# Farmadupe/vid_dup_finder_lib

Measured on AMD Instinct MI355X. Metric: hash-pairs/sec all-pairs Hamming (search(), tolerance 0.35) [+ frames/sec DCT-hash in 'summary.hash_summary'], higher is better.
Workload: dtype fp4 e2m1 ({0,1}) x fp4 -> f32 accumulate (exact half-integers < 2^11)

## Files before the change

### vid_dup_finder_lib_amd/csrc/api.cpp

```cpp
#include <algorithm>
#include <chrono>
#include <cmath>
#include <cstdio>
#include <cstdlib>
#include <cstring>
#include <memory>
#include <numeric>

#include "host_sort.h"
#include "vdf_ctx.h"

namespace {
thread_local std::string g_create_error;
inline double now_ms() { return std::chrono::duration<double, std::milli>(std::chrono::steady_clock::now().time_since_epoch()).count(); }
}

vdf_ctx::~vdf_ctx()
{
    if (!subs.empty() || !workers.empty()) vdf_impl::destroy_multi(this);
    if (copy_pool) vdf_impl::destroy_copy_pool(this);
    for (auto &kv : axis_tables) {
        kv.second->start.release(); kv.second->size.release(); kv.second->w.release();
        delete kv.second;
    }
    for (auto &kv : mfma_tables) {
        kv.second->operand.release(); kv.second->bias.release(); kv.second->meta.release();
        delete kv.second;
    }
    for (auto &kv : box_tables) {
        kv.second->blob.release(); kv.second->entries.release();
        delete kv.second;
    }
    DevBuf *all[] = {&row_lo, &row_hi, &tile_lo, &tile_hi, &tile_first, &tile_count, &tile_offset, &counters,
                     &hits, &perm, &matched, &exp_cols, &exp_rows, &pop_cols, &pop_rows, &cand, &group_cmin, &group_offset, &group_blocks, &up_hashes,
                     &up_dur, &up_ref_hashes, &up_ref_dur, &small, &frames, &frames2, &out_hashes, &out_hashes2, &out_dc,
                     &out_dc2, &cos_table, &crops, &crop_desc, &crop_tables, &crop_desc2, &crop_tables2, &crop_work, &sort_scratch, &sort_scratch_pub, &hits2, &hit_bitmaps, &bitmap_gather};
    for (DevBuf *b : all) b->release();
    for (PinBuf &b : pin) b.release();
    for (PinBuf &b : pin_out) b.release();
    pin_small.release();
    pin_ctrl.release();
    pin_crops.release();
    pin_desc.release();
    host_hits.buf.release();
    if (ev0) (void)hipEventDestroy(ev0);
    if (ev1) (void)hipEventDestroy(ev1);
    if (ev_mid) (void)hipEventDestroy(ev_mid);
    if (ev_wait) (void)hipEventDestroy(ev_wait);
    for (hipEvent_t e : ev_copy) if (e) (void)hipEventDestroy(e);
    for (hipEvent_t e : ev_done) if (e) (void)hipEventDestroy(e);
    if (copy_stream) (void)hipStreamDestroy(copy_stream);
    if (stream) (void)hipStreamDestroy(stream);
}

namespace vdf_impl {

void set_create_error(const std::string &msg) { g_create_error = msg; }

int fail(vdf_ctx *ctx, int code, const std::string &msg)
{
    if (ctx) ctx->err = msg;
    return code;
}

int fail_hip(vdf_ctx *ctx, hipError_t e, const char *what)
{
    std::string msg = std::string(what) + ": " + hipGetErrorString(e);
    (void)hipGetLastError();
    return fail(ctx, e == hipErrorOutOfMemory ? VDF_E_OOM : VDF_E_HIP, msg);
}

bool is_sorted_u32(const uint32_t *d, size_t n)
{
    for (size_t i = 1; i < n; i++)
        if (d[i] < d[i - 1]) return false;
    return true;
}

constexpr size_t kPinSmallBytes = 4u << 20;
constexpr uint64_t kDeviceSortHits = 1u << 17;
constexpr uint32_t kRefsMinWorkgroups = 2048;
constexpr uint64_t kSpecSortHits = 1u << 14;
constexpr uint64_t kFilterHits = 1u << 16;

int search_core(vdf_ctx *ctx, int mode, const uint64_t *d_col_hashes, const uint32_t *d_col_dur, size_t n_cols,
                const uint64_t *d_row_hashes, const uint32_t *d_row_dur, const uint32_t *d_row_perm, size_t n_rows,
                uint32_t tol_int, uint32_t shard_index, uint32_t shard_count, uint32_t row_begin, uint32_t row_end,
                const uint32_t *d_matched, uint32_t row_index_base, vdf_hit *hits, uint64_t capacity,
                uint64_t *n_hits_out, uint32_t *overflow_row_out, hipStream_t stream, bool replay_only, vdf_ctx::HostHits *staging,
                ShardExchange *fx)
{
    *n_hits_out = 0;
    *overflow_row_out = 0xFFFFFFFFu;
    if (n_rows == 0 || n_cols == 0) return VDF_OK;
    if (n_rows >= 0xFFFFFFFFull || n_cols >= 0xFFFFFFFFull) return fail(ctx, VDF_E_INVAL, "more than 2^32-1 hashes");
    if (shard_count == 0 || shard_index >= shard_count) return fail(ctx, VDF_E_INVAL, "bad shard index/count");
    VDF_HIP(ctx, hipSetDevice(ctx->device));
    const double t_enter = now_ms();

    vdf::SearchLaunch L{};
    const bool mfma = ctx->search_backend == 1;
    L.tile_rows = mfma ? (mode == 1 ? ctx->mfma_refs_rows : ctx->mfma_self_rows) : ctx->tile_rows;
    L.chunk_cols = mfma ? ctx->mfma_chunk_cols : ctx->chunk_cols;
    L.n_row_tiles = (uint32_t)((n_rows + L.tile_rows - 1) / L.tile_rows);
    if (mfma && L.chunk_cols == 0) {
        L.chunk_cols = 65536;
        while (L.chunk_cols > 4096 && (uint64_t)L.n_row_tiles * ((n_cols + L.chunk_cols - 1) / L.chunk_cols) < ctx->mfma_min_wgs) L.chunk_cols /= 2;
    }
    while ((uint64_t)L.n_row_tiles * ((n_cols + L.chunk_cols - 1) / L.chunk_cols) >= 0x40000000ull && L.chunk_cols < (1u << 22))
        L.chunk_cols *= 2;
    const size_t padded_rows = (size_t)L.n_row_tiles * L.tile_rows;
    VDF_HIP(ctx, ctx->row_lo.reserve(padded_rows * 4));
    VDF_HIP(ctx, ctx->row_hi.reserve(padded_rows * 4));
    VDF_HIP(ctx, ctx->tile_lo.reserve((size_t)L.n_row_tiles * 4));
    VDF_HIP(ctx, ctx->tile_hi.reserve((size_t)L.n_row_tiles * 4));
    VDF_HIP(ctx, ctx->tile_first.reserve((size_t)L.n_row_tiles * 4));
    VDF_HIP(ctx, ctx->tile_count.reserve((size_t)L.n_row_tiles * 4));
    VDF_HIP(ctx, ctx->tile_offset.reserve(((size_t)L.n_row_tiles + 1) * 4));
    VDF_HIP(ctx, ctx->counters.reserve(64));
    const uint64_t dev_cap = std::max<uint64_t>(capacity, 1);
    VDF_HIP(ctx, ctx->hits.reserve(dev_cap * sizeof(vdf_hit)));

    L.row_hashes = reinterpret_cast<const uint32_t *>(d_row_hashes);
    L.row_perm = d_row_perm;
    L.n_rows = (uint32_t)n_rows;
    L.row_index_base = row_index_base;
    L.col_hashes = reinterpret_cast<const uint32_t *>(d_col_hashes);
    L.n_cols = (uint32_t)n_cols;
    L.row_lo = ctx->row_lo.as<uint32_t>();
    L.row_hi = ctx->row_hi.as<uint32_t>();
    L.tile_lo = ctx->tile_lo.as<uint32_t>();
    L.tile_hi = ctx->tile_hi.as<uint32_t>();
    L.tile_first = ctx->tile_first.as<uint32_t>();
    L.tile_count = ctx->tile_count.as<uint32_t>();
    L.tile_offset = ctx->tile_offset.as<uint32_t>();
    L.tol = tol_int;
    L.matched = d_matched;
    L.self_mode = (mode == 0);
    L.shard_index = shard_index;
    L.shard_count = shard_count;
    L.hits = ctx->hits.as<vdf_hit>();
    L.capacity = capacity;
    L.counters = ctx->counters.as<unsigned long long>();
    L.overflow_row = reinterpret_cast<uint32_t *>(ctx->counters.as<unsigned long long>() + 4);

    L.prune_step = 16;
    if (ctx->mfma_prune_step >= 0) {
        L.prune_step = ctx->mfma_prune_step;
    } else {
        for (int st = 6; st <= 14; st++) {
            const double bits = 64.0 * (st + 1);
            if (bits / 2 - 2.0 * std::sqrt(bits) >= (double)tol_int + 1) { L.prune_step = st; break; }
        }
    }
    if (mfma) L.prune_step = L.prune_step <= 6 ? 6 : L.prune_step <= 8 ? 8 : L.prune_step <= 10 ? 10 : L.prune_step <= 14 ? L.prune_step : 16;
    else L.prune_step = L.prune_step <= 6 ? 6 : L.prune_step <= 10 ? 10 : L.prune_step <= 12 ? 12 : 16;
    if (mfma) {
        L.group_size = std::min<uint32_t>(ctx->mfma_group, L.n_row_tiles);
        L.n_groups = (L.n_row_tiles + L.group_size - 1) / L.group_size;
        if (L.n_groups > 1024) return fail(ctx, VDF_E_INVAL, "too many row-tile groups");
        VDF_HIP(ctx, ctx->group_cmin.reserve((size_t)L.n_groups * 4));
        VDF_HIP(ctx, ctx->group_offset.reserve(((size_t)L.n_groups + 1) * 4));
        VDF_HIP(ctx, ctx->group_blocks.reserve((size_t)L.n_groups * 4));
        L.group_blocks = ctx->group_blocks.as<uint32_t>();
        L.group_cmin = ctx->group_cmin.as<uint32_t>();
        L.group_offset = ctx->group_offset.as<uint32_t>();
        const uint32_t k_steps = (uint32_t)(L.prune_step < 15 ? L.prune_step + 1 : 16);
        const uint32_t col_pad = (uint32_t)((n_cols + vdf::kMfmaRowPad - 1) / vdf::kMfmaRowPad * vdf::kMfmaRowPad) + vdf::kMfmaColPad;
        VDF_HIP(ctx, ctx->exp_cols.reserve((size_t)col_pad * 512));
        VDF_HIP(ctx, ctx->pop_cols.reserve((size_t)col_pad * 12));
        const ExpOwner want_owner{d_col_hashes, n_cols, k_steps, ctx->exp_cols.p};
        const bool reuse = ctx->pinned_db == d_col_hashes && ctx->pinned_n == n_cols && ctx->exp_owner == want_owner;
        if (!reuse) {
            ctx->exp_owner = ExpOwner{};
            VDF_HIP(ctx, vdf::launch_expand_fp4(L.col_hashes, (uint32_t)n_cols, col_pad, ctx->exp_cols.p, k_steps,
                                                ctx->pop_cols.as<float>(), stream));
            ctx->exp_owner = want_owner;
        }
        L.col_exp = ctx->exp_cols.p;
        L.col_pop3 = ctx->pop_cols.as<float>();
        L.col_pad = col_pad;
        if (d_row_hashes == d_col_hashes) {
            L.row_exp = ctx->exp_cols.p;
            L.row_pop3 = L.col_pop3;
            L.row_pad = col_pad;
        } else {
            const uint32_t row_pad = (uint32_t)((padded_rows + 127) / 128 * 128);
            VDF_HIP(ctx, ctx->exp_rows.reserve((size_t)row_pad * 512));
            VDF_HIP(ctx, ctx->pop_rows.reserve((size_t)row_pad * 12));
            VDF_HIP(ctx, vdf::launch_expand_fp4(L.row_hashes, (uint32_t)n_rows, row_pad, ctx->exp_rows.p, k_steps,
                                                ctx->pop_rows.as<float>(), stream));
            L.row_exp = ctx->exp_rows.p;
            L.row_pop3 = ctx->pop_rows.as<float>();
            L.row_pad = row_pad;
        }
    }
    const unsigned long long init[8] = {0, 0, 0, 0, 0xFFFFFFFFull, 0, 0, 0};
    const bool pin_ok = ctx->pin_small.reserve(kPinSmallBytes) && ctx->pin_small.pinned;
    uint64_t spec = std::min<uint64_t>(capacity, std::max<uint64_t>(ctx->hits_guess + ctx->hits_guess / 4 + 1024, 8192));
    if (!pin_ok || spec * sizeof(vdf_hit) > kPinSmallBytes) spec = 0;
    const bool spec_sort = spec && ctx->hits_guess >= kSpecSortHits;
    if (spec_sort) VDF_HIP(ctx, hipMemsetAsync(ctx->hits.p, 0xFF, (size_t)spec * sizeof(vdf_hit), stream));
    const bool adapt_refs = mode == 1 && mfma && ctx->mfma_chunk_cols == 0;
    if (adapt_refs && ctx->refs_hint_cols == n_cols && ctx->refs_hint_rows == n_rows && ctx->refs_hint_chunk) L.chunk_cols = ctx->refs_hint_chunk;
    if (!ctx->pin_ctrl.reserve(256)) return fail(ctx, VDF_E_OOM, "pinned staging");
    unsigned long long *pre = ctx->pin_ctrl.as<unsigned long long>() + 8;
    uint32_t total_tiles = 0;
    unsigned long long unsorted = 0, admitted = 0;
    for (int pass = 0;; pass++) {
        VDF_HIP(ctx, hipMemcpyAsync(ctx->counters.p, init, sizeof init, hipMemcpyHostToDevice, stream));
        VDF_HIP(ctx, vdf::launch_windows_tiles(mode, d_col_dur, (uint32_t)n_cols, d_row_dur, d_row_perm, (uint32_t)n_rows,
                                               row_begin, row_end, shard_index, shard_count, L, stream));
        VDF_HIP(ctx, hipMemcpyAsync(pre, L.counters, 64, hipMemcpyDeviceToHost, stream));
        VDF_HIP(ctx, hipMemcpyAsync(pre + 8, mfma ? L.group_offset + L.n_groups : L.tile_offset + L.n_row_tiles, 4,
                                    hipMemcpyDeviceToHost, stream));
        VDF_HIP(ctx, hipMemcpyAsync(pre + 9, L.tile_offset + L.n_row_tiles, 4, hipMemcpyDeviceToHost, stream));
        VDF_HIP(ctx, hipStreamSynchronize(stream));
        total_tiles = *reinterpret_cast<const uint32_t *>(pre + 8);
        const uint32_t busy_tiles = *reinterpret_cast<const uint32_t *>(pre + 9);
        unsorted = pre[5];
        admitted = pre[2];
        if (!adapt_refs || pass > 0 || unsorted || busy_tiles == 0 || busy_tiles >= kRefsMinWorkgroups || L.chunk_cols <= 4096) break;
        uint64_t est = busy_tiles;
        while (L.chunk_cols > 4096 && est < kRefsMinWorkgroups) { L.chunk_cols /= 2; est *= 2; }
    }
    if (adapt_refs) { ctx->refs_hint_cols = n_cols; ctx->refs_hint_rows = n_rows; ctx->refs_hint_chunk = L.chunk_cols; }
    if (unsorted) return fail(ctx, VDF_E_INVAL, "durations are not ascending: pass the arrays in Search::sort order");
    if (total_tiles >= 0x7FFFFFFFu) return fail(ctx, VDF_E_INVAL, "tile count exceeds the grid limit");
    if (mfma) {
        const uint64_t want = ((uint64_t)((double)admitted * 6e-6) + (uint64_t)total_tiles * 8 * 8 + std::max<uint64_t>(capacity, 1ull << 20)) * ctx->cand_scale;
        L.cand_capacity = (uint32_t)std::min<uint64_t>(want, 0x40000000ull);
        if (ctx->cand_capacity_override)
            L.cand_capacity = (uint32_t)std::min<uint64_t>((uint64_t)ctx->cand_capacity_override * ctx->cand_scale, 0x40000000ull);
        const void *before = ctx->cand.p;
        VDF_HIP(ctx, ctx->cand.reserve((size_t)L.cand_capacity * 16));
        if (ctx->cand.p != before) ctx->cand_dirty = SIZE_MAX;
        const size_t slots = ctx->cand.cap / 16;
        const size_t fill = (ctx->cand_dirty == SIZE_MAX ? slots : std::min<size_t>(slots, ctx->cand_dirty)) * 16;
        if (fill) VDF_HIP(ctx, hipMemsetAsync(ctx->cand.p, 0xFF, fill, stream));
        ctx->cand_dirty = L.cand_capacity;
        L.cand = ctx->cand.p;
        L.cand_head = ctx->counters.as<unsigned long long>() + 6;
    }

    ctx->timing.prep_ms += (float)(now_ms() - t_enter);
    VDF_HIP(ctx, hipEventRecord(ctx->ev0, stream));
    if (mfma) {
        VDF_HIP(ctx, vdf::launch_hamming_tiles_mfma2(L, total_tiles, stream));
        VDF_HIP(ctx, hipEventRecord(ctx->ev_mid, stream));
        if (total_tiles) VDF_HIP(ctx, vdf::launch_resolve_candidates(L, stream));
    } else {
        VDF_HIP(ctx, vdf::launch_hamming_tiles(L, total_tiles, stream));
        VDF_HIP(ctx, hipEventRecord(ctx->ev_mid, stream));
    }
    VDF_HIP(ctx, hipEventRecord(ctx->ev1, stream));
    if (!ctx->pin_ctrl.reserve(256)) return fail(ctx, VDF_E_OOM, "pinned staging");
    unsigned long long *fin = ctx->pin_ctrl.as<unsigned long long>();
    VDF_HIP(ctx, hipMemcpyAsync(fin, ctx->counters.p, 64, hipMemcpyDeviceToHost, stream));
    unsigned row_bits = 1;
    while (row_bits < 32 && ((uint64_t)row_index_base + n_rows) >> row_bits) row_bits++;
    unsigned col_bits = 1;
    while (col_bits < 32 && ((uint64_t)n_cols >> col_bits)) col_bits++;
    if (spec_sort) {
        VDF_HIP(ctx, ctx->sort_scratch.reserve(vdf::sort_hits_scratch_bytes((size_t)spec)));
        VDF_HIP(ctx, vdf::launch_sort_hits(ctx->hits.as<vdf_hit>(), (size_t)spec, row_bits, ctx->sort_scratch.p, ctx->sort_scratch.cap, stream, col_bits));
    }
    if (spec) VDF_HIP(ctx, hipMemcpyAsync(ctx->pin_small.p, ctx->hits.p, (size_t)spec * sizeof(vdf_hit), hipMemcpyDeviceToHost, stream));
    VDF_HIP(ctx, hipStreamSynchronize(stream));
    const double t_synced = now_ms();
    float ms = 0.f, ms_stream = 0.f;
    VDF_HIP(ctx, hipEventElapsedTime(&ms, ctx->ev0, ctx->ev1));
// ... 1465 lines not shown
```

### vid_dup_finder_lib_amd/csrc/hamming.hip

```cpp
#include <algorithm>

#include "vdf_internal.h"

namespace vdf {

constexpr uint32_t kMaxBlocksPerLaunch = 4u << 20;

typedef const __attribute__((address_space(4))) uint32_t *const_u32_ptr;

__device__ __forceinline__ uint32_t sat_u32(double x)
{
    if (!(x == x)) return 0u;
    if (x <= 0.0) return 0u;
    if (x >= 4294967295.0) return 0xFFFFFFFFu;
    return (uint32_t)x;
}

__device__ __forceinline__ uint32_t partition_point_lt(const uint32_t *__restrict__ d, uint32_t n, uint32_t v)
{
    uint32_t lo = 0, hi = n;
    while (lo < hi) {
        uint32_t mid = lo + ((hi - lo) >> 1);
        if (d[mid] < v) lo = mid + 1; else hi = mid;
    }
    return lo;
}
__device__ __forceinline__ uint32_t partition_point_le(const uint32_t *__restrict__ d, uint32_t n, uint32_t v)
{
    uint32_t lo = 0, hi = n;
    while (lo < hi) {
        uint32_t mid = lo + ((hi - lo) >> 1);
        if (d[mid] <= v) lo = mid + 1; else hi = mid;
    }
    return lo;
}

__device__ __forceinline__ uint32_t wave_min(uint32_t v)
{
#pragma unroll
    for (int o = 32; o > 0; o >>= 1) v = min(v, (uint32_t)__shfl_xor((int)v, o, 64));
    return v;
}
__device__ __forceinline__ uint32_t wave_max(uint32_t v)
{
#pragma unroll
    for (int o = 32; o > 0; o >>= 1) v = max(v, (uint32_t)__shfl_xor((int)v, o, 64));
    return v;
}

__device__ __forceinline__ void wave_append_hits(bool hit, uint32_t row, uint32_t col, vdf_hit *__restrict__ hits,
                                                 unsigned long long capacity, unsigned long long *__restrict__ counters,
                                                 uint32_t *__restrict__ overflow_row)
{
    const unsigned long long bal = __builtin_amdgcn_ballot_w64(hit);
    if (bal == 0ull) return;
    const int leader = __builtin_ctzll(bal);
    unsigned long long base = 0;
    if ((int)(threadIdx.x & 63) == leader) base = atomicAdd(&counters[0], (unsigned long long)__builtin_popcountll(bal));
    base = ((unsigned long long)(uint32_t)__shfl((int)(base >> 32), leader, 64) << 32) | (uint32_t)__shfl((int)(uint32_t)base, leader, 64);
    if (hit) {
        const unsigned long long at = base + __builtin_amdgcn_mbcnt_hi((uint32_t)(bal >> 32), __builtin_amdgcn_mbcnt_lo((uint32_t)bal, 0u));
        if (at < capacity) {
            vdf_hit hp; hp.row = row; hp.col = col;
            hits[at] = hp;
        } else {
            atomicMin(overflow_row, row);
        }
    }
}

__global__ __launch_bounds__(256) void windows_tiles_kernel(
    int mode, const uint32_t *__restrict__ col_dur, uint32_t n_cols, const uint32_t *__restrict__ row_dur,
    const uint32_t *__restrict__ row_perm, uint32_t n_rows, uint32_t row_begin, uint32_t row_end, uint32_t shard_index,
    uint32_t shard_count, uint32_t tile_rows, uint32_t chunk_cols, uint32_t *__restrict__ row_lo,
    uint32_t *__restrict__ row_hi, uint32_t *__restrict__ tile_lo, uint32_t *__restrict__ tile_hi,
    uint32_t *__restrict__ tile_first, uint32_t *__restrict__ tile_count, unsigned long long *__restrict__ counters)
{
    __shared__ uint32_t s_min[4], s_max[4];
    __shared__ unsigned long long s_pairs[4];
    const uint32_t t = blockIdx.x;
    const bool mine = (t % shard_count) == shard_index;
    uint32_t mn = 0xFFFFFFFFu, mx = 0u;
    unsigned long long pairs = 0;
    for (uint32_t q = threadIdx.x; q < tile_rows; q += 256) {
// ... 156 lines not shown
#pragma unroll
            for (int q = 0; q < 8; q++) {
                const uint4 v = rp[q];
                rw[k][4 * q + 0] = v.x; rw[k][4 * q + 1] = v.y; rw[k][4 * q + 2] = v.z; rw[k][4 * q + 3] = v.w;
            }
            if (self_mode && matched && ((matched[src >> 5] >> (src & 31)) & 1u)) { lo = 0; hi = 0; }
        } else {
#pragma unroll
            for (int q = 0; q < 32; q++) rw[k][q] = 0u;
            lo = 0; hi = 0;
        }
        rlo[k] = lo; rhi[k] = hi; rid[k] = row_index_base + src;
    }

    const_u32_ptr cols = (const_u32_ptr)(uintptr_t)col_hashes;
    uint32_t n_early = 0;
    for (uint32_t c = c_begin; c < c_end; ++c) {
        const_u32_ptr cp = cols + (size_t)c * 32;
        uint32_t d[R];
#pragma unroll
        for (int k = 0; k < R; k++) d[k] = 0u;
#pragma unroll
        for (int w = 0; w < (CHKW < 32 ? CHKW : 32); ++w) {
            const uint32_t cw = cp[w];
#pragma unroll
            for (int k = 0; k < R; k++) d[k] += __builtin_popcount(rw[k][w] ^ cw);
        }
        uint32_t m = d[0];
#pragma unroll
        for (int k = 1; k < R; k++) m = min(m, d[k]);
        if (CHKW < 32) {
            if (__builtin_amdgcn_ballot_w64(m <= tol) == 0ull) { n_early += 1; continue; }
#pragma unroll
            for (int w = CHKW; w < 32; ++w) {
                const uint32_t cw = cp[w];
#pragma unroll
                for (int k = 0; k < R; k++) d[k] += __builtin_popcount(rw[k][w] ^ cw);
            }
            m = d[0];
#pragma unroll
            for (int k = 1; k < R; k++) m = min(m, d[k]);
        }
        if (__builtin_amdgcn_ballot_w64(m <= tol) != 0ull) {
            bool col_ok = true;
            if (matched) col_ok = ((((const_u32_ptr)(uintptr_t)matched)[c >> 5] >> (c & 31)) & 1u) == 0u;
            if (col_ok) {
#pragma unroll
                for (int k = 0; k < R; k++)
                    wave_append_hits(d[k] <= tol && c >= rlo[k] && c < rhi[k], rid[k], c, hits, capacity, counters, overflow_row);
            }
        }
    }
    if (threadIdx.x == 0) atomicAdd(&counters[1], (unsigned long long)(c_end - c_begin) * TILE_ROWS);
    if (CHKW < 32 && lane == 0 && n_early) atomicAdd(&counters[3], (unsigned long long)n_early * (64u * R));
}

typedef int v8i __attribute__((ext_vector_type(8)));
typedef int v4i __attribute__((ext_vector_type(4)));
typedef float v16f __attribute__((ext_vector_type(16)));

__global__ __launch_bounds__(256) void expand_fp4_kernel(const uint32_t *__restrict__ packed, uint32_t n,
                                                        uint32_t n_pad, uint4 *__restrict__ expanded,
                                                        uint32_t k_steps, float *__restrict__ pop,
                                                        float *__restrict__ popk, float *__restrict__ popkT)
{
    for (size_t idx = (size_t)blockIdx.x * 256 + threadIdx.x; idx < (size_t)n_pad * 32;
         idx += (size_t)gridDim.x * 256) {
    const uint32_t hsh = (uint32_t)(idx >> 5), dw = (uint32_t)idx & 31u;
    uint4 out = {0u, 0u, 0u, 0u};
    uint32_t w = 0;
    if (hsh < n) {
        w = packed[idx];
        uint32_t o[4];
#pragma unroll
        for (int j = 0; j < 4; j++) {
            uint32_t x = (w >> (8 * j)) & 0xFFu;
            x = (x | (x << 12)) & 0x000F000Fu;
            x = (x | (x << 6)) & 0x03030303u;
            x = (x | (x << 3)) & 0x11111111u;
            o[j] = x << 1;
        }
        out = make_uint4(o[0], o[1], o[2], o[3]);
    }
    expanded[idx] = out;
    if (pop) {
        uint32_t pc = (uint32_t)__builtin_popcount(w), pk = (dw & 15u) < k_steps ? pc : 0u;
#pragma unroll
        for (int o = 16; o > 0; o >>= 1) { pc += (uint32_t)__shfl_xor((int)pc, o, 32); pk += (uint32_t)__shfl_xor((int)pk, o, 32); }
        if (dw == 0) {
            pop[hsh] = (float)pc;
            popk[hsh] = (float)pk;
            popkT[(size_t)(hsh >> 7) * 128 + (hsh & 31u) * 4 + ((hsh >> 5) & 3u)] = (float)pk;
        }
    }
    }
}

template <int N>
struct IntC { static constexpr int value = N; };
template <int I, int N, class F>
__device__ __forceinline__ void static_for(F &&f)
{
    if constexpr (I < N) {
        f(IntC<I>{});
        static_for<I + 1, N>(f);
    }
}

struct CandEntry {
    uint32_t row_base;
    uint32_t col;
    uint32_t mask;
    uint32_t pad;
};

__global__ __launch_bounds__(256) void resolve_candidates_kernel(
    const CandEntry *__restrict__ cand, const unsigned long long *__restrict__ cand_head, uint32_t cand_capacity,
    const uint32_t *__restrict__ row_hashes, const uint32_t *__restrict__ row_perm, uint32_t n_rows, uint32_t row_index_base,
    const uint32_t *__restrict__ col_hashes, uint32_t n_cols, const uint32_t *__restrict__ row_lo,
    const uint32_t *__restrict__ row_hi, uint32_t tol, const uint32_t *__restrict__ matched, int self_mode,
    vdf_hit *__restrict__ hits, unsigned long long capacity, unsigned long long *__restrict__ counters,
    uint32_t *__restrict__ overflow_row)
{
    const uint32_t n = (uint32_t)min(*cand_head, (unsigned long long)cand_capacity);
    const uint32_t lane = threadIdx.x & 63, wave = threadIdx.x >> 6;
    constexpr uint32_t kStage = 512;
    __shared__ vdf_hit s_stage[4][kStage];
    uint32_t staged = 0;
    auto flush = [&]() {
        if (staged == 0) return;
        __builtin_amdgcn_fence(__ATOMIC_ACQ_REL, "wavefront");
        __builtin_amdgcn_wave_barrier();
        unsigned long long base = 0;
        if (lane == 0) base = atomicAdd(&counters[0], (unsigned long long)staged);
        base = ((unsigned long long)(uint32_t)__builtin_amdgcn_readfirstlane((int)(base >> 32)) << 32) |
               (uint32_t)__builtin_amdgcn_readfirstlane((int)(uint32_t)base);
        for (uint32_t k = lane; k < staged; k += 64) {
            const vdf_hit hp = s_stage[wave][k];
            if (base + k < capacity) hits[base + k] = hp;
            else atomicMin(overflow_row, hp.row);
        }
        __builtin_amdgcn_fence(__ATOMIC_ACQ_REL, "wavefront");
        __builtin_amdgcn_wave_barrier();
        staged = 0;
    };
    for (uint32_t e0 = blockIdx.x * 256 + (threadIdx.x & ~63u); e0 < n; e0 += gridDim.x * 256) {
        const uint32_t e = e0 + lane;
        CandEntry ce;
        ce.row_base = 0xFFFFFFFFu; ce.col = 0; ce.mask = 0; ce.pad = 0;
        if (e < n) ce = cand[e];
        uint32_t m = ce.mask;
        if (ce.row_base == 0xFFFFFFFFu || ce.col >= n_cols) m = 0;
        if (m && matched && ((matched[ce.col >> 5] >> (ce.col & 31)) & 1u)) m = 0;
        uint4 cw[8];
        if (m) {
            const uint4 *cp = reinterpret_cast<const uint4 *>(col_hashes + (size_t)ce.col * 32);
#pragma unroll
            for (int q = 0; q < 8; q++) cw[q] = cp[q];
        }
        while (__builtin_amdgcn_ballot_w64(m != 0u) != 0ull) {
            bool hit = false;
            uint32_t src = 0;
            if (m) {
                const uint32_t r = (uint32_t)__builtin_ctz(m);
                m &= m - 1;
                const uint32_t p = ce.row_base + (r & 3) + 8 * (r >> 2);
                if (p < n_rows) {
                    const uint32_t lo = row_lo[p], hi = row_hi[p];
                    if (ce.col >= lo && ce.col < hi) {
                        src = row_perm ? row_perm[p] : p;
                        if (!(self_mode && matched && ((matched[src >> 5] >> (src & 31)) & 1u))) {
                            const uint4 *rp = reinterpret_cast<const uint4 *>(row_hashes + (size_t)src * 32);
                            uint32_t d = 0;
#pragma unroll
                            for (int q = 0; q < 8; q++) {
                                const uint4 v = rp[q];
                                d += __builtin_popcount(v.x ^ cw[q].x) + __builtin_popcount(v.y ^ cw[q].y) +
                                     __builtin_popcount(v.z ^ cw[q].z) + __builtin_popcount(v.w ^ cw[q].w);
                            }
                            hit = d <= tol;
                        }
                    }
                }
            }
            const unsigned long long bal = __builtin_amdgcn_ballot_w64(hit);
            if (bal == 0ull) continue;
            const uint32_t cnt = (uint32_t)__builtin_popcountll(bal);
            if (staged + cnt > kStage) flush();
            if (hit) {
                vdf_hit hp; hp.row = row_index_base + src; hp.col = ce.col;
                s_stage[wave][staged + __builtin_amdgcn_mbcnt_hi((uint32_t)(bal >> 32), __builtin_amdgcn_mbcnt_lo((uint32_t)bal, 0u))] = hp;
            }
            staged += cnt;
        }
    }
    flush();
}

template <int CHK, int WAVES>
__global__ __launch_bounds__(64 * WAVES, 2) void hamming_mfma2_kernel(
    const uint4 *__restrict__ row_exp, const uint32_t *__restrict__ row_perm, uint32_t n_rows,
    uint32_t row_index_base, const uint4 *__restrict__ col_exp, const uint32_t *__restrict__ row_lo,
    const uint32_t *__restrict__ row_hi, const uint32_t *__restrict__ tile_lo, const uint32_t *__restrict__ tile_hi,
    const uint32_t *__restrict__ tile_first, const uint32_t *__restrict__ tile_count,
    const uint32_t *__restrict__ group_offset, const uint32_t *__restrict__ group_cmin, uint32_t n_groups,
    uint32_t group_size, uint32_t shard_index, uint32_t shard_count, uint32_t n_row_tiles, uint32_t chunk_cols,
    uint32_t tol, const uint32_t *__restrict__ matched, int self_mode, vdf_hit *__restrict__ hits,
    unsigned long long capacity, unsigned long long *__restrict__ counters, uint32_t *__restrict__ overflow_row,
    uint32_t block_base, const float *__restrict__ row_pop3, uint32_t row_pad, const float *__restrict__ col_pop3,
    uint32_t col_pad, CandEntry *__restrict__ cand, uint32_t cand_capacity, unsigned long long *__restrict__ cand_head)
{
    constexpr int K = CHK < 15 ? CHK + 1 : 16;
    constexpr bool kRowcLds = K > 13;
    constexpr uint32_t kSub = WAVES >= 8 ? 4 : 2;
    constexpr uint32_t kColStep = 32 * kSub;
    constexpr int NBLK = 2 * (int)kSub;
    constexpr int NM = NBLK * K;
    constexpr int P = (K == 16 && WAVES >= 8) ? 2 : 4, NB = P + 1;
    constexpr uint32_t kTileRows = 64 * WAVES;
    constexpr int kDmaPerWave = (int)(kColStep * 32 / (64 * WAVES));
    constexpr int kDmaEvery = NM / kDmaPerWave;
    static_assert(kDmaEvery >= 2, "stage too short for its DMA pieces");
    constexpr int kTestAt = 2;
    static_assert(K >= kTestAt + 4, "block too short to hide the previous block's test");
    const uint32_t bid = blockIdx.x + block_base;
    __shared__ __attribute__((aligned(16))) uint4 s_b0[kColStep * 32];
    __shared__ __attribute__((aligned(16))) uint4 s_b1[kColStep * 32];
    const uint32_t tid = threadIdx.x, lane = tid & 63, g = lane >> 5, c31 = lane & 31;
    const uint32_t wave = (uint32_t)__builtin_amdgcn_readfirstlane((int)(tid >> 6));

    const_u32_ptr goff = (const_u32_ptr)(uintptr_t)group_offset;
    uint32_t gl = 0, gh = n_groups;
    while (gh - gl > 1) {
        const uint32_t mid = (gl + gh) >> 1;
        if (goff[mid] <= bid) gl = mid; else gh = mid;
    }
    const uint32_t idx = bid - goff[gl];
    const uint32_t per_group = (group_size + shard_count - 1) / shard_count;
    const uint32_t g0 = gl * group_size;
    const uint32_t t0 = g0 + (shard_index + shard_count - g0 % shard_count) % shard_count;
    const uint32_t t = t0 + (idx % per_group) * shard_count;
    const uint32_t chunk = ((const_u32_ptr)(uintptr_t)group_cmin)[gl] + idx / per_group;
    if (t >= n_row_tiles || t >= g0 + group_size) return;
    {
        const uint32_t f = ((const_u32_ptr)(uintptr_t)tile_first)[t], cnt = ((const_u32_ptr)(uintptr_t)tile_count)[t];
        if (chunk < f || chunk >= f + cnt) return;
    }
    const uint32_t t_lo = ((const_u32_ptr)(uintptr_t)tile_lo)[t];
    const uint32_t t_hi = ((const_u32_ptr)(uintptr_t)tile_hi)[t];
    const uint32_t c_begin = max(chunk * chunk_cols, t_lo);
    const uint32_t c_end = min((chunk + 1) * chunk_cols, t_hi);
    if (c_begin >= c_end) return;

    const float tol_f = (float)min(tol, 1024u);
    const float *row_popk = row_pop3 + row_pad;
    const float *col_popkT = col_pop3 + 2 * (size_t)col_pad;
    const uint32_t row0 = t * kTileRows + wave * 64;
    v4i a[2][K];
    const float4 *s_rc = nullptr;
    v16f rowc[2];
    uint32_t live[2];
#pragma unroll
    for (int rt = 0; rt < 2; rt++) {
        live[rt] = 0;
        const uint32_t p = row0 + 32 * rt + c31;
        uint32_t src = p;
        if (p < n_rows && row_perm) src = row_perm[p];
        const uint4 *rp = row_exp + (size_t)src * 32 + 16 * g;
#pragma unroll
        for (int s = 0; s < K; s++) {
            const uint4 v = rp[s];
            a[rt][s] = (v4i){(int)v.x, (int)v.y, (int)v.z, (int)v.w};
        }
#pragma unroll
        for (int r = 0; r < 16; r++) {
            const uint32_t pr = row0 + 32 * rt + (r & 3) + 8 * (r >> 2) + 4 * g;
            const uint32_t sr = (pr < n_rows && row_perm) ? row_perm[pr] : pr;
            rowc[rt][r] = -0.5f * row_popk[sr];
            if (row_hi[pr] > row_lo[pr]) live[rt] |= 1u << r;
        }
    }
    if constexpr (kRowcLds) {
        __shared__ __attribute__((aligned(16))) float4 s_rowc[WAVES * 2 * 2 * 4];
        float4 *mine = s_rowc + ((size_t)wave * 2 * 2 + g) * 4;
        if (c31 == 0) {
#pragma unroll
            for (int rt = 0; rt < 2; rt++)
#pragma unroll
                for (int q = 0; q < 4; q++)
                    mine[rt * 2 * 4 + q] = float4{rowc[rt][4 * q], rowc[rt][4 * q + 1], rowc[rt][4 * q + 2], rowc[rt][4 * q + 3]};
        }
        s_rc = mine;
    }
    const uint32_t cb0 = c_begin & ~(kColStep - 1);
    constexpr uint32_t kColsPerRound = 2 * WAVES;
    constexpr int kOffsets = 32 / kColsPerRound;
    static_assert(kOffsets >= 1 && (kOffsets & (kOffsets - 1)) == 0, "piece addressing");
    const uint32_t c0 = 2 * wave + g;
    uint32_t lane_off[kOffsets];
#pragma unroll
    for (int j = 0; j < kOffsets; j++) lane_off[j] = c0 * 512u + ((((lane & 31) ^ c0) << 4) ^ (16u * kColsPerRound * j));
    auto stage_rsrc = [&](uint32_t cb) __attribute__((always_inline)) {
        return __builtin_amdgcn_make_buffer_rsrc(
            const_cast<char *>(reinterpret_cast<const char *>(col_exp) + (size_t)cb * 512), 0, kColStep * 512u, 0x00020000);
    };
    auto load_piece = [&](__amdgpu_buffer_rsrc_t rs, uint4 *dst, int i) __attribute__((always_inline)) {
        auto *lds = (__attribute__((address_space(3))) void *)&dst[64 * WAVES * i + 64 * wave];
        const int voff = (int)lane_off[i & (kOffsets - 1)], soff = (int)(512u * kColsPerRound * (uint32_t)i);
        __builtin_amdgcn_raw_ptr_buffer_load_lds(rs, lds, 16, voff, soff, 0, 0);
    };
    auto load_thr = [&](uint32_t cb, float (&out)[kSub]) __attribute__((always_inline)) {
        const float *q = col_popkT + (size_t)(cb >> 7) * 128 + c31 * 4 + ((cb >> 5) & 3u);
        if constexpr (kSub == 4) {
            const float4 v = *reinterpret_cast<const float4 *>(q);
            out[0] = v.x; out[1] = v.y; out[2] = v.z; out[3] = v.w;
        } else {
            const float2 v = *reinterpret_cast<const float2 *>(q);
            out[0] = v.x; out[1] = v.y;
        }
    };

    v16f acc[2] = {v16f{}, v16f{}};
    if constexpr (kRowcLds) acc[0] = rowc[0];
    uint32_t n_early = 0;
    float thr[kSub], thr_next[kSub];

    constexpr uint32_t kCandChunk = 8, kCandChunkMax = 512;
    uint32_t q_chunk = kCandChunk, q_taken = 0;
    unsigned long long q_next = 0, q_end = 0;
    auto emit = [&](const v16f &c, float thrv, uint32_t live_rows, uint32_t rows_first, uint32_t col_first) __attribute__((always_inline)) {
        uint32_t mask = 0;
#pragma unroll
        for (int r = 0; r < 16; r++) mask |= (c[r] >= thrv) ? (1u << r) : 0u;
        mask &= live_rows;
        const uint32_t j = col_first + c31;
        if (j < c_begin || j >= c_end) mask = 0;
        const unsigned long long bal = __builtin_amdgcn_ballot_w64(mask != 0u);
        if (bal == 0ull) return;
        const uint32_t need = (uint32_t)__builtin_popcountll(bal);
        if (q_next + need > q_end) {
            if (q_taken >= 2) q_chunk = min(2u * q_chunk, kCandChunkMax);
            q_taken++;
            const uint32_t take = max((need + kCandChunk - 1) / kCandChunk * kCandChunk, q_chunk);
            unsigned long long base = 0;
            if (lane == 0) base = atomicAdd(cand_head, (unsigned long long)take);
            q_next = ((unsigned long long)(uint32_t)__builtin_amdgcn_readfirstlane((int)(base >> 32)) << 32) |
                     (uint32_t)__builtin_amdgcn_readfirstlane((int)(uint32_t)base);
            q_end = q_next + take;
        }
        const unsigned long long slot = q_next + __builtin_amdgcn_mbcnt_hi((uint32_t)(bal >> 32), __builtin_amdgcn_mbcnt_lo((uint32_t)bal, 0u));
        if (mask != 0u) {
            if (slot < cand_capacity) {
                CandEntry ce; ce.row_base = rows_first + 4 * g; ce.col = j; ce.mask = mask; ce.pad = 0;
                *reinterpret_cast<uint4 *>(&cand[slot]) = *reinterpret_cast<const uint4 *>(&ce);
            } else {
                const uint32_t p = rows_first + 4 * g + (uint32_t)(__builtin_ctz(mask) & 3) + 8 * (uint32_t)(__builtin_ctz(mask) >> 2);
                if (p < n_rows) atomicMin(overflow_row, row_index_base + (row_perm ? row_perm[p] : p));
            }
        }
        q_next += need;
    };

    auto run_stage = [&](uint32_t cb, const uint4 *cur, uint4 *nxt) __attribute__((always_inline)) {
        const uint32_t cb_next = cb + kColStep < c_end ? cb + kColStep : cb;
        const __amdgpu_buffer_rsrc_t rs_next = stage_rsrc(cb_next);
        load_thr(cb_next, thr_next);
        uint32_t flags = 0;
        uint4 fq[NB];
        auto frag = [&](int i) __attribute__((always_inline)) {
            const uint32_t sub = (uint32_t)((i / K) >> 1), s = (uint32_t)(i % K);
            return cur[((32u * sub + c31) << 5) | ((s + 16u * g) ^ c31)];
        };
#pragma unroll
        for (int i = 0; i < P; i++) fq[i] = frag(i);
        __builtin_amdgcn_sched_barrier(0);
        float m0 = 0.f, m1 = 0.f, m2 = 0.f, m3 = 0.f, m4 = 0.f, m5 = 0.f;
        static_for<0, NM>([&](auto ic) __attribute__((always_inline)) {
            constexpr int i = decltype(ic)::value;
            constexpr int blk = i / K, s = i % K, rt = blk & 1;
            const uint4 bv = fq[i % NB];
            const v8i b = {(int)bv.x, (int)bv.y, (int)bv.z, (int)bv.w, 0, 0, 0, 0};
            const v8i ar = {a[rt][s].x, a[rt][s].y, a[rt][s].z, a[rt][s].w, 0, 0, 0, 0};
            if constexpr (s == 0 && !kRowcLds) acc[rt] = __builtin_amdgcn_mfma_scale_f32_32x32x64_f8f6f4(ar, b, rowc[rt], 4, 4, 0, 0, 0, 0);
            else acc[rt] = __builtin_amdgcn_mfma_scale_f32_32x32x64_f8f6f4(ar, b, acc[rt], 4, 4, 0, 0, 0, 0);
            if constexpr (i + P < NM) fq[(i + P) % NB] = frag(i + P);
            if constexpr ((i % kDmaEvery) == 1 && (i / kDmaEvery) < kDmaPerWave) load_piece(rs_next, nxt, i / kDmaEvery);
            if constexpr (blk >= 1) {
                const v16f &c = acc[rt ^ 1];
                if constexpr (s == kTestAt) {
                    m0 = fmaxf(fmaxf(c[0], c[1]), c[2]); m1 = fmaxf(fmaxf(c[3], c[4]), c[5]); m2 = fmaxf(fmaxf(c[6], c[7]), c[8]);
                } else if constexpr (s == kTestAt + 1) {
                    m3 = fmaxf(fmaxf(c[9], c[10]), c[11]); m4 = fmaxf(fmaxf(c[12], c[13]), c[14]);
                } else if constexpr (s == kTestAt + 2) {
                    m5 = fmaxf(fmaxf(m0, m1), m2); m3 = fmaxf(fmaxf(m3, m4), c[15]);
                } else if constexpr (s == kTestAt + 3) {
                    if (__builtin_amdgcn_ballot_w64(fmaxf(m5, m3) >= thr[(blk - 1) >> 1]) != 0ull) {
                        flags |= 1u << (blk - 1);
                        emit(c, thr[(blk - 1) >> 1], live[rt ^ 1], row0 + 32u * (uint32_t)(rt ^ 1), cb + 32u * (uint32_t)((blk - 1) >> 1));
                    }
                }
            }
            if constexpr (kRowcLds && s >= kTestAt + 4 && s < kTestAt + 8) {
                constexpr int q = s - (kTestAt + 4);
                const float4 v = s_rc[((rt ^ 1) * 2) * 4 + q];
                acc[rt ^ 1][4 * q + 0] = v.x; acc[rt ^ 1][4 * q + 1] = v.y; acc[rt ^ 1][4 * q + 2] = v.z; acc[rt ^ 1][4 * q + 3] = v.w;
            }
            __builtin_amdgcn_sched_barrier(0);
        });
        {
            const v16f &c = acc[(NBLK - 1) & 1];
            m0 = fmaxf(fmaxf(c[0], c[1]), c[2]); m1 = fmaxf(fmaxf(c[3], c[4]), c[5]); m2 = fmaxf(fmaxf(c[6], c[7]), c[8]);
            m3 = fmaxf(fmaxf(c[9], c[10]), c[11]); m4 = fmaxf(fmaxf(c[12], c[13]), c[14]);
            const float pm = fmaxf(fmaxf(fmaxf(m0, m1), m2), fmaxf(fmaxf(m3, m4), c[15]));
            if (__builtin_amdgcn_ballot_w64(pm >= thr[kSub - 1]) != 0ull) {
                flags |= 1u << (NBLK - 1);
                emit(c, thr[kSub - 1], live[(NBLK - 1) & 1], row0 + 32u * (uint32_t)((NBLK - 1) & 1), cb + 32u * (kSub - 1));
            }
        }
        uint32_t valid = 0;
#pragma unroll
        for (uint32_t sub = 0; sub < kSub; sub++)
            if (cb + 32u * sub < c_end) valid |= 3u << (2 * sub);
        flags &= valid;
        n_early += (uint32_t)__builtin_popcount(valid & ~flags);
        asm volatile("s_waitcnt vmcnt(0)" ::: "memory");
        __syncthreads();
#pragma unroll
        for (uint32_t sub = 0; sub < kSub; sub++) thr[sub] = 0.5f * (thr_next[sub] - tol_f);
    };

#pragma unroll
    for (int i = 0; i < kDmaPerWave; i++) load_piece(stage_rsrc(cb0), s_b0, i);
    load_thr(cb0, thr_next);
#pragma unroll
    for (int rt = 0; rt < 2; rt++)
#pragma unroll
        for (int s = 0; s < K; s++) asm volatile("" ::"v"(a[rt][s]));
    asm volatile("s_waitcnt vmcnt(0)" ::: "memory");
    __syncthreads();
#pragma unroll
    for (uint32_t sub = 0; sub < kSub; sub++) thr[sub] = 0.5f * (thr_next[sub] - tol_f);
    for (uint32_t cb = cb0; cb < c_end; cb += 2 * kColStep) {
        run_stage(cb, s_b0, s_b1);
        if (cb + kColStep >= c_end) break;
        run_stage(cb + kColStep, s_b1, s_b0);
    }
    if (tid == 0) atomicAdd(&counters[1], (unsigned long long)(c_end - c_begin) * kTileRows);
    if (CHK < 15 && lane == 0 && n_early) atomicAdd(&counters[3], (unsigned long long)n_early * (32u * 32u));
}

__global__ __launch_bounds__(256) void hits_mark_incoming_kernel(const vdf_hit *__restrict__ hits, unsigned long long n,
                                                                 uint32_t *__restrict__ has_in)
{
    for (size_t i = (size_t)blockIdx.x * 256 + threadIdx.x; i < n; i += (size_t)gridDim.x * 256) {
        const uint32_t j = hits[i].col;
        if (!((has_in[j >> 5] >> (j & 31)) & 1u)) atomicOr(&has_in[j >> 5], 1u << (j & 31));
    }
}

__global__ __launch_bounds__(256) void hits_mark_covered_kernel(const vdf_hit *__restrict__ hits, unsigned long long n,
                                                                const uint32_t *__restrict__ has_in, uint32_t *__restrict__ covered)
{
    for (size_t i = (size_t)blockIdx.x * 256 + threadIdx.x; i < n; i += (size_t)gridDim.x * 256) {
        const vdf_hit h = hits[i];
        if (!((has_in[h.row >> 5] >> (h.row & 31)) & 1u) && !((covered[h.col >> 5] >> (h.col & 31)) & 1u))
            atomicOr(&covered[h.col >> 5], 1u << (h.col & 31));
    }
}

__global__ __launch_bounds__(256) void hits_compact_kernel(const vdf_hit *__restrict__ hits, unsigned long long n,
                                                           const uint32_t *__restrict__ covered, vdf_hit *__restrict__ out,
                                                           unsigned long long *__restrict__ counter)
{
    const size_t n_round = (n + 63) & ~(size_t)63;
    for (size_t i = (size_t)blockIdx.x * 256 + threadIdx.x; i < n_round; i += (size_t)gridDim.x * 256) {
        vdf_hit h{0u, 0u};
        bool keep = false;
        if (i < n) {
            h = hits[i];
            keep = !((covered[h.row >> 5] >> (h.row & 31)) & 1u);
        }
        const unsigned long long bal = __builtin_amdgcn_ballot_w64(keep);
        if (bal == 0ull) continue;
        const int leader = __builtin_ctzll(bal);
        unsigned long long base = 0;
        if ((int)(threadIdx.x & 63) == leader) base = atomicAdd(counter, (unsigned long long)__builtin_popcountll(bal));
        base = ((unsigned long long)(uint32_t)__shfl((int)(base >> 32), leader, 64) << 32) | (uint32_t)__shfl((int)(uint32_t)base, leader, 64);
        if (keep) out[base + __builtin_amdgcn_mbcnt_hi((uint32_t)(bal >> 32), __builtin_amdgcn_mbcnt_lo((uint32_t)bal, 0u))] = h;
    }
}

__global__ __launch_bounds__(256) void bitmap_or_kernel(uint32_t *__restrict__ dst, const uint32_t *__restrict__ srcs, size_t n_words,
                                                        uint32_t n_srcs)
{
    for (size_t w = (size_t)blockIdx.x * 256 + threadIdx.x; w < n_words; w += (size_t)gridDim.x * 256) {
        uint32_t v = dst[w];
        for (uint32_t r = 0; r < n_srcs; r++) v |= srcs[(size_t)r * n_words + w];
        dst[w] = v;
    }
}

hipError_t launch_bitmap_or(uint32_t *dst, const uint32_t *srcs, size_t n_words, uint32_t n_srcs, hipStream_t stream)
{
    if (n_words == 0 || n_srcs == 0) return hipSuccess;
    const uint32_t grid = (uint32_t)std::min<size_t>((n_words + 255) / 256, 4096);
    hipLaunchKernelGGL(bitmap_or_kernel, dim3(grid), dim3(256), 0, stream, dst, srcs, n_words, n_srcs);
    return hipGetLastError();
}

static inline uint32_t filter_grid(unsigned long long n_hits) { return (uint32_t)std::min<unsigned long long>(std::max<unsigned long long>((n_hits + 255) / 256, 1ull), 8192ull); }

hipError_t launch_filter_mark_incoming(const vdf_hit *hits, unsigned long long n_hits, uint32_t n_entries, uint32_t *bitmaps, hipStream_t stream)
{
    const size_t words = ((size_t)n_entries + 31) / 32;
    hipError_t e = hipMemsetAsync(bitmaps, 0, 2 * words * 4, stream);
    if (e != hipSuccess) return e;
    if (n_hits) hipLaunchKernelGGL(hits_mark_incoming_kernel, dim3(filter_grid(n_hits)), dim3(256), 0, stream, hits, n_hits, bitmaps);
    return hipGetLastError();
}

hipError_t launch_filter_mark_covered(const vdf_hit *hits, unsigned long long n_hits, uint32_t n_entries, uint32_t *bitmaps, hipStream_t stream)
{
    const size_t words = ((size_t)n_entries + 31) / 32;
    if (n_hits) hipLaunchKernelGGL(hits_mark_covered_kernel, dim3(filter_grid(n_hits)), dim3(256), 0, stream, hits, n_hits, bitmaps, bitmaps + words);
    return hipGetLastError();
}

hipError_t launch_filter_compact(const vdf_hit *hits, unsigned long long n_hits, uint32_t n_entries, const uint32_t *bitmaps, vdf_hit *out,
// ... 161 lines not shown
```

Before: 4562 billion.

## Store only pruned k-steps of expanded hashes and add three-deep LDS stage ring

The expanded fp4 column and row hashes now hold only the k_steps chunks the pruned kernel actually reads, not all 32 chunks. This shrinks global storage, DMA volume and LDS per stage, and a new rotation swizzle keeps LDS access free of bank conflicts. When LDS has room (8 waves), a three-buffer ring prefetches two stages ahead and carries fragment prefetch across stage boundaries. The cost is more complex addressing and extra LDS, and the CHK=15/full path must stay consistent with the compacted layout.

```diff
diff --git a/vid_dup_finder_lib_amd/csrc/api.cpp b/vid_dup_finder_lib_amd/csrc/api.cpp
--- a/vid_dup_finder_lib_amd/csrc/api.cpp
+++ b/vid_dup_finder_lib_amd/csrc/api.cpp
@@ -8,6 +8,7 @@
 #include <numeric>
 
 #include "host_sort.h"
+#include "search_stage_layout.h"
 #include "vdf_ctx.h"
 
 namespace {
@@ -167,7 +168,7 @@
         L.group_offset = ctx->group_offset.as<uint32_t>();
         const uint32_t k_steps = (uint32_t)(L.prune_step < 15 ? L.prune_step + 1 : 16);
         const uint32_t col_pad = (uint32_t)((n_cols + vdf::kMfmaRowPad - 1) / vdf::kMfmaRowPad * vdf::kMfmaRowPad) + vdf::kMfmaColPad;
-        VDF_HIP(ctx, ctx->exp_cols.reserve((size_t)col_pad * 512));
+        VDF_HIP(ctx, ctx->exp_cols.reserve((size_t)col_pad * vdf::stage::hash_bytes(k_steps)));
         VDF_HIP(ctx, ctx->pop_cols.reserve((size_t)col_pad * 12));
         const ExpOwner want_owner{d_col_hashes, n_cols, k_steps, ctx->exp_cols.p};
         const bool reuse = ctx->pinned_db == d_col_hashes && ctx->pinned_n == n_cols && ctx->exp_owner == want_owner;
@@ -186,7 +187,7 @@
             L.row_pad = col_pad;
         } else {
             const uint32_t row_pad = (uint32_t)((padded_rows + 127) / 128 * 128);
-            VDF_HIP(ctx, ctx->exp_rows.reserve((size_t)row_pad * 512));
+            VDF_HIP(ctx, ctx->exp_rows.reserve((size_t)row_pad * vdf::stage::hash_bytes(k_steps)));
             VDF_HIP(ctx, ctx->pop_rows.reserve((size_t)row_pad * 12));
             VDF_HIP(ctx, vdf::launch_expand_fp4(L.row_hashes, (uint32_t)n_rows, row_pad, ctx->exp_rows.p, k_steps,
                                                 ctx->pop_rows.as<float>(), stream));
diff --git a/vid_dup_finder_lib_amd/csrc/hamming.hip b/vid_dup_finder_lib_amd/csrc/hamming.hip
--- a/vid_dup_finder_lib_amd/csrc/hamming.hip
+++ b/vid_dup_finder_lib_amd/csrc/hamming.hip
@@ -1,5 +1,6 @@
 #include <algorithm>
 
+#include "search_stage_layout.h"
 #include "vdf_internal.h"
 
 namespace vdf {
@@ -322,7 +323,7 @@
         }
         out = make_uint4(o[0], o[1], o[2], o[3]);
     }
-    expanded[idx] = out;
+    if ((dw & 15u) < k_steps) expanded[(size_t)hsh * stage::chunks(k_steps) + stage::chunk_of_dword(k_steps, dw)] = out;
     if (pop) {
         uint32_t pc = (uint32_t)__builtin_popcount(w), pk = (dw & 15u) < k_steps ? pc : 0u;
 #pragma unroll
@@ -458,14 +459,22 @@
     constexpr int NM = NBLK * K;
     constexpr int P = (K == 16 && WAVES >= 8) ? 2 : 4, NB = P + 1;
     constexpr uint32_t kTileRows = 64 * WAVES;
-    constexpr int kDmaPerWave = (int)(kColStep * 32 / (64 * WAVES));
-    constexpr int kDmaEvery = NM / kDmaPerWave;
-    static_assert(kDmaEvery >= 2, "stage too short for its DMA pieces");
+    static_assert(stage::valid(K, WAVES) && kColStep == stage::cols(WAVES), "stage layout");
+    constexpr uint32_t J = stage::chunks(K);
+    constexpr int kRing = (int)stage::ring_depth(K, WAVES);
+    constexpr int kDmaRounds = (int)stage::rounds(K, WAVES);
+    constexpr int kDmaEvery = (int)stage::dma_every(K, WAVES, NM);
+    static_assert(kDmaEvery >= 2 && (kDmaRounds - 1) * kDmaEvery + 1 < NM, "stage too short for its DMA pieces");
     constexpr int kTestAt = 2;
     static_assert(K >= kTestAt + 4, "block too short to hide the previous block's test");
     const uint32_t bid = blockIdx.x + block_base;
-    __shared__ __attribute__((aligned(16))) uint4 s_b0[kColStep * 32];
-    __shared__ __attribute__((aligned(16))) uint4 s_b1[kColStep * 32];
+    __shared__ __attribute__((aligned(16))) uint4 s_b0[kColStep * J];
+    __shared__ __attribute__((aligned(16))) uint4 s_b1[kColStep * J];
+    uint4 *s_b2 = nullptr;
+    if constexpr (kRing >= 3) {
+        __shared__ __attribute__((aligned(16))) uint4 s_b2_[kColStep * J];
+        s_b2 = s_b2_;
+    }
     const uint32_t tid = threadIdx.x, lane = tid & 63, g = lane >> 5, c31 = lane & 31;
     const uint32_t wave = (uint32_t)__builtin_amdgcn_readfirstlane((int)(tid >> 6));
 
@@ -506,7 +515,7 @@
         const uint32_t p = row0 + 32 * rt + c31;
         uint32_t src = p;
         if (p < n_rows && row_perm) src = row_perm[p];
-        const uint4 *rp = row_exp + (size_t)src * 32 + 16 * g;
+        const uint4 *rp = row_exp + (size_t)src * J + K * g;
 #pragma unroll
         for (int s = 0; s < K; s++) {
             const uint4 v = rp[s];
@@ -533,21 +542,22 @@
         s_rc = mine;
     }
     const uint32_t cb0 = c_begin & ~(kColStep - 1);
-    constexpr uint32_t kColsPerRound = 2 * WAVES;
-    constexpr int kOffsets = 32 / kColsPerRound;
-    static_assert(kOffsets >= 1 && (kOffsets & (kOffsets - 1)) == 0, "piece addressing");
-    const uint32_t c0 = 2 * wave + g;
-    uint32_t lane_off[kOffsets];
-#pragma unroll
-    for (int j = 0; j < kOffsets; j++) lane_off[j] = c0 * 512u + ((((lane & 31) ^ c0) << 4) ^ (16u * kColsPerRound * j));
     auto stage_rsrc = [&](uint32_t cb) __attribute__((always_inline)) {
         return __builtin_amdgcn_make_buffer_rsrc(
-            const_cast<char *>(reinterpret_cast<const char *>(col_exp) + (size_t)cb * 512), 0, kColStep * 512u, 0x00020000);
+            const_cast<char *>(reinterpret_cast<const char *>(col_exp) + (size_t)cb * stage::hash_bytes(K)), 0, kColStep * stage::hash_bytes(K), 0x00020000);
     };
-    auto load_piece = [&](__amdgpu_buffer_rsrc_t rs, uint4 *dst, int i) __attribute__((always_inline)) {
-        auto *lds = (__attribute__((address_space(3))) void *)&dst[64 * WAVES * i + 64 * wave];
-        const int voff = (int)lane_off[i & (kOffsets - 1)], soff = (int)(512u * kColsPerRound * (uint32_t)i);
-        __builtin_amdgcn_raw_ptr_buffer_load_lds(rs, lds, 16, voff, soff, 0, 0);
+    auto load_piece = [&](__amdgpu_buffer_rsrc_t rs, uint4 *dst, int round) __attribute__((always_inline)) {
+        constexpr uint32_t kWavesIn[8] = {stage::waves_in_round(K, WAVES, 0), stage::waves_in_round(K, WAVES, 1), stage::waves_in_round(K, WAVES, 2),
+                                          stage::waves_in_round(K, WAVES, 3), stage::waves_in_round(K, WAVES, 4), stage::waves_in_round(K, WAVES, 5),
+                                          stage::waves_in_round(K, WAVES, 6), stage::waves_in_round(K, WAVES, 7)};
+        static_assert(kDmaRounds <= 8, "piece rounds");
+        if (kWavesIn[round] == WAVES || wave < kWavesIn[round]) {
+            auto *lds = (__attribute__((address_space(3))) void *)&dst[64 * WAVES * round + 64 * wave];
+            uint32_t slot0 = tid;
+            asm volatile("" : "+v"(slot0));
+            const int voff = (int)stage::source_offset_of_slot(K, 64u * WAVES * (uint32_t)round + slot0);
+            __builtin_amdgcn_raw_ptr_buffer_load_lds(rs, lds, 16, voff, 0, 0, 0);
+        }
     };
     auto load_thr = [&](uint32_t cb, float (&out)[kSub]) __attribute__((always_inline)) {
         const float *q = col_popkT + (size_t)(cb >> 7) * 128 + c31 * 4 + ((cb >> 5) & 3u);
@@ -601,18 +611,22 @@
         q_next += need;
     };
 
-    auto run_stage = [&](uint32_t cb, const uint4 *cur, uint4 *nxt) __attribute__((always_inline)) {
+    const uint32_t frag_chunk0 = stage::lane_chunk0(K, c31, g), frag_base = stage::lane_base(K, c31, g);
+    auto frag = [&](const uint4 *buf, int i) __attribute__((always_inline)) {
+        return buf[stage::frag_slot(K, (uint32_t)((i / K) >> 1), (uint32_t)(i % K), frag_base, frag_chunk0)];
+    };
+    uint4 fq[NB];
+
+    auto run_stage = [&](uint32_t cb, const uint4 *cur, const uint4 *ahead, uint4 *fill) __attribute__((always_inline)) {
         const uint32_t cb_next = cb + kColStep < c_end ? cb + kColStep : cb;
-        const __amdgpu_buffer_rsrc_t rs_next = stage_rsrc(cb_next);
+        const uint32_t cb_fill = kRing >= 3 ? (cb + 2 * kColStep < c_end ? cb + 2 * kColStep : cb) : cb_next;
+        const __amdgpu_buffer_rsrc_t rs_fill = stage_rsrc(cb_fill);
         load_thr(cb_next, thr_next);
         uint32_t flags = 0;
-        uint4 fq[NB];
-        auto frag = [&](int i) __attribute__((always_inline)) {
-            const uint32_t sub = (uint32_t)((i / K) >> 1), s = (uint32_t)(i % K);
-            return cur[((32u * sub + c31) << 5) | ((s + 16u * g) ^ c31)];
-        };
-#pragma unroll
-        for (int i = 0; i < P; i++) fq[i] = frag(i);
+        if constexpr (kRing < 3) {
+#pragma unroll
+            for (int i = 0; i < P; i++) fq[i] = frag(cur, i);
+        }
         __builtin_amdgcn_sched_barrier(0);
         float m0 = 0.f, m1 = 0.f, m2 = 0.f, m3 = 0.f, m4 = 0.f, m5 = 0.f;
         static_for<0, NM>([&](auto ic) __attribute__((always_inline)) {
@@ -623,8 +637,9 @@
             const v8i ar = {a[rt][s].x, a[rt][s].y, a[rt][s].z, a[rt][s].w, 0, 0, 0, 0};
             if constexpr (s == 0 && !kRowcLds) acc[rt] = __builtin_amdgcn_mfma_scale_f32_32x32x64_f8f6f4(ar, b, rowc[rt], 4, 4, 0, 0, 0, 0);
             else acc[rt] = __builtin_amdgcn_mfma_scale_f32_32x32x64_f8f6f4(ar, b, acc[rt], 4, 4, 0, 0, 0, 0);
-            if constexpr (i + P < NM) fq[(i + P) % NB] = frag(i + P);
-            if constexpr ((i % kDmaEvery) == 1 && (i / kDmaEvery) < kDmaPerWave) load_piece(rs_next, nxt, i / kDmaEvery);
+            if constexpr (i + P < NM) fq[(i + P) % NB] = frag(cur, i + P);
+            else if constexpr (kRing >= 3) fq[(i + P) % NB] = frag(ahead, i + P - NM);
+            if constexpr ((i % kDmaEvery) == 1 && (i / kDmaEvery) < kDmaRounds) load_piece(rs_fill, fill, i / kDmaEvery);
             if constexpr (blk >= 1) {
                 const v16f &c = acc[rt ^ 1];
                 if constexpr (s == kTestAt) {
@@ -667,10 +682,22 @@
         __syncthreads();
 #pragma unroll
         for (uint32_t sub = 0; sub < kSub; sub++) thr[sub] = 0.5f * (thr_next[sub] - tol_f);
+        if constexpr (kRing >= 3 && NM % NB != 0) {
+            uint4 t[P];
+#pragma unroll
+            for (int i = 0; i < P; i++) t[i] = fq[(NM + i) % NB];
+#pragma unroll
+            for (int i = 0; i < P; i++) fq[i] = t[i];
+        }
     };
 
 #pragma unroll
-    for (int i = 0; i < kDmaPerWave; i++) load_piece(stage_rsrc(cb0), s_b0, i);
+    for (int i = 0; i < kDmaRounds; i++) load_piece(stage_rsrc(cb0), s_b0, i);
+    if constexpr (kRing >= 3) {
+        const __amdgpu_buffer_rsrc_t rs1 = stage_rsrc(cb0 + kColStep < c_end ? cb0 + kColStep : cb0);
+#pragma unroll
+        for (int i = 0; i < kDmaRounds; i++) load_piece(rs1, s_b1, i);
+    }
     load_thr(cb0, thr_next);
 #pragma unroll
     for (int rt = 0; rt < 2; rt++)
@@ -680,10 +707,22 @@
     __syncthreads();
 #pragma unroll
     for (uint32_t sub = 0; sub < kSub; sub++) thr[sub] = 0.5f * (thr_next[sub] - tol_f);
-    for (uint32_t cb = cb0; cb < c_end; cb += 2 * kColStep) {
-        run_stage(cb, s_b0, s_b1);
-        if (cb + kColStep >= c_end) break;
-        run_stage(cb + kColStep, s_b1, s_b0);
+    if constexpr (kRing >= 3) {
+#pragma unroll
+        for (int i = 0; i < P; i++) fq[i] = frag(s_b0, i);
+        for (uint32_t cb = cb0; cb < c_end; cb += 3 * kColStep) {
+            run_stage(cb, s_b0, s_b1, s_b2);
+            if (cb + kColStep >= c_end) break;
+            run_stage(cb + kColStep, s_b1, s_b2, s_b0);
+            if (cb + 2 * kColStep >= c_end) break;
+            run_stage(cb + 2 * kColStep, s_b2, s_b0, s_b1);
+        }
+    } else {
+        for (uint32_t cb = cb0; cb < c_end; cb += 2 * kColStep) {
+            run_stage(cb, s_b0, s_b1, s_b1);
+            if (cb + kColStep >= c_end) break;
+            run_stage(cb + kColStep, s_b1, s_b0, s_b0);
+        }
     }
     if (tid == 0) atomicAdd(&counters[1], (unsigned long long)(c_end - c_begin) * kTileRows);
     if (CHK < 15 && lane == 0 && n_early) atomicAdd(&counters[3], (unsigned long long)n_early * (32u * 32u));
diff --git a/vid_dup_finder_lib_amd/csrc/search_stage_layout.h b/vid_dup_finder_lib_amd/csrc/search_stage_layout.h
--- /dev/null
+++ b/vid_dup_finder_lib_amd/csrc/search_stage_layout.h
@@ -0,0 +1,95 @@
+#pragma once
+#include <cstdint>
+
+namespace vdf {
+namespace stage {
+
+constexpr uint32_t kLdsBytesPerCu = 163840;
+constexpr uint32_t kPieceSlots = 64;
+
+constexpr uint32_t k_steps_of(int chk) { return chk < 15 ? (uint32_t)chk + 1u : 16u; }
+
+constexpr uint32_t chunks(uint32_t K) { return 2u * K; }
+constexpr uint32_t hash_bytes(uint32_t K) { return 16u * chunks(K); }
+constexpr uint32_t chunk_of_dword(uint32_t K, uint32_t dw) { return (dw >> 4) * K + (dw & 15u); }
+
+constexpr uint32_t cols(uint32_t waves) { return waves >= 8 ? 128u : 64u;  }
+constexpr uint32_t stage_slots(uint32_t K, uint32_t waves) { return cols(waves) * chunks(K); }
+constexpr uint32_t stage_bytes(uint32_t K, uint32_t waves) { return 16u * stage_slots(K, waves); }
+
+constexpr uint32_t rot_classes(uint32_t K)
+{
+    const uint32_t j = chunks(K);
+    return (j % 16u) == 0 ? 16u : (j % 8u) == 0 ? 8u : (j % 4u) == 0 ? 4u : 2u;
+}
+constexpr uint32_t rot_shift(uint32_t K)
+{
+    const uint32_t period = 16u / rot_classes(K);
+    return period == 8 ? 3u : period == 4 ? 2u : period == 2 ? 1u : 0u;
+}
+constexpr uint32_t max_rotation(uint32_t K) { return rot_classes(K) - 1u; }
+constexpr uint32_t rotation(uint32_t K, uint32_t col) { return (col >> rot_shift(K)) & max_rotation(K); }
+constexpr uint32_t slot(uint32_t K, uint32_t col, uint32_t j)
+{
+    return chunks(K) == 32u ? 32u * col + (j ^ (col & 31u)) : chunks(K) * col + (j + rotation(K, col)) % chunks(K);
+}
+
+constexpr uint32_t lane_chunk0(uint32_t K, uint32_t c31, uint32_t g) { return chunks(K) == 32u ? (16u * g) ^ c31 : K * g + rotation(K, c31); }
+constexpr uint32_t lane_base(uint32_t K, uint32_t c31, uint32_t g) { return chunks(K) == 32u ? 32u * c31 : chunks(K) * c31 + lane_chunk0(K, c31, g); }
+constexpr bool may_wrap(uint32_t K, uint32_t s) { return s + max_rotation(K) >= K; }
+constexpr uint32_t frag_slot(uint32_t K, uint32_t sub, uint32_t s, uint32_t base, uint32_t chunk0)
+{
+    if (chunks(K) == 32u) return 32u * 32u * sub + (base | (s ^ chunk0));
+    uint32_t at = base + s;
+    if (may_wrap(K, s) && chunk0 + s >= chunks(K)) at -= chunks(K);
+    return 32u * chunks(K) * sub + at;
+}
+
+constexpr uint32_t pieces(uint32_t K, uint32_t waves) { return stage_slots(K, waves) / kPieceSlots; }
+constexpr uint32_t rounds(uint32_t K, uint32_t waves) { return (pieces(K, waves) + waves - 1u) / waves; }
+constexpr uint32_t waves_in_round(uint32_t K, uint32_t waves, uint32_t round)
+{
+    const uint32_t left = pieces(K, waves) - round * waves;
+    return left < waves ? left : waves;
+}
+constexpr uint32_t source_offset_of_slot(uint32_t K, uint32_t L)
+{
+    if (chunks(K) == 32u) return 16u * ((L & ~31u) | ((L ^ (L >> 5)) & 31u));
+    const uint32_t J = chunks(K), col = L / J, r = L - col * J, rot = rotation(K, col);
+    return 16u * (L - rot + (r < rot ? J : 0u));
+}
+constexpr uint32_t source_offset(uint32_t K, uint32_t piece, uint32_t lane) { return source_offset_of_slot(K, kPieceSlots * piece + lane); }
+
+#ifndef VDF_STAGE_RING_MAX
+#define VDF_STAGE_RING_MAX 3
+#endif
+constexpr uint32_t other_lds_bytes(uint32_t K, uint32_t waves) { return K > 13 ? waves * 64u : 0u; }
+constexpr uint32_t workgroups_per_cu(uint32_t waves) { return waves >= 8 ? 1u : 2u; }
+constexpr uint32_t ring_depth(uint32_t K, uint32_t waves)
+{
+    return (VDF_STAGE_RING_MAX >= 3 && waves >= 8 && 3u * stage_bytes(K, waves) + other_lds_bytes(K, waves) <= kLdsBytesPerCu) ? 3u : 2u;
+}
+constexpr uint32_t lds_bytes_per_cu(uint32_t K, uint32_t waves)
+{
+    return workgroups_per_cu(waves) * (ring_depth(K, waves) * stage_bytes(K, waves) + other_lds_bytes(K, waves));
+}
+
+#ifndef VDF_STAGE_DMA_SPAN_NUM
+#define VDF_STAGE_DMA_SPAN_NUM 2
+#define VDF_STAGE_DMA_SPAN_DEN 3
+#endif
+constexpr uint32_t dma_every(uint32_t K, uint32_t waves, uint32_t mfmas_per_stage)
+{
+    const uint32_t span = ring_depth(K, waves) >= 3 ? mfmas_per_stage * VDF_STAGE_DMA_SPAN_NUM / VDF_STAGE_DMA_SPAN_DEN : mfmas_per_stage;
+    return span / rounds(K, waves);
+}
+
+constexpr bool valid(uint32_t K, uint32_t waves)
+{
+    return K >= 1 && K <= 16 && (waves == 8 || waves == 4) && stage_slots(K, waves) % kPieceSlots == 0 &&
+           rot_shift(K) + (rot_classes(K) == 16 ? 4u : rot_classes(K) == 8 ? 3u : rot_classes(K) == 4 ? 2u : 1u) <= 4u &&
+           lds_bytes_per_cu(K, waves) <= kLdsBytesPerCu;
+}
+
+}
+}
```

After: 4438 billion. 0.973x the previous value.
